# onolab-tmu/overiva

Measured on AMD Instinct MI355X. Metric: AuxIVA iterations/sec (2048 bins x 4000 frames x 8 mics), higher is better.
Workload: dtype f32

## Files before the change

include/overiva_hip.h:

```cpp
#ifndef OVERIVA_HIP_H
#define OVERIVA_HIP_H

#ifdef __cplusplus
extern "C" {
#endif

#define OIVA_OK 0
#define OIVA_ERR_ARG (-1)
#define OIVA_ERR_HIP (-2)
#define OIVA_ERR_STATE (-3)
#define OIVA_ERR_NUMERIC (-4)

#define OIVA_MODEL_LAPLACE 0
#define OIVA_MODEL_GAUSS 1

#define OIVA_MAX_CHANNELS 32

#define OIVA_PREC_FAST 0
#define OIVA_PREC_UPDATE_F64 1
#define OIVA_PREC_UPDATE_ROWS 2
#define OIVA_PREC_COV_F64 4
#define OIVA_PREC_PRECISE (OIVA_PREC_UPDATE_F64 | OIVA_PREC_COV_F64)

typedef struct oiva_plan oiva_plan;
// ... 49 lines not shown
int oiva_plan_save_w(oiva_plan *p);
int oiva_plan_restore_w(oiva_plan *p);

int oiva_plan_iterate_timed(oiva_plan *p, int n, float *total_ms, float *per_kernel_ms);
#define OIVA_N_STAGES 4

int oiva_plan_get_cov_splits(oiva_plan *p, int *nsplit);
int oiva_plan_set_cov_splits(oiva_plan *p, int nsplit);
int oiva_plan_set_cov_quad(oiva_plan *p, int enable, int *active);
int oiva_plan_set_pow_splits(oiva_plan *p, int nsplit);
int oiva_plan_set_cov_hmfma(oiva_plan *p, int enable);
int oiva_plan_set_fuse_cov_update(oiva_plan *p, int enable, int *active);
int oiva_plan_set_power_reverse(oiva_plan *p, int enable);
int oiva_plan_set_x_resident_mb(oiva_plan *p, double mb);
int oiva_plan_get_x_resident(oiva_plan *p, int *n16, int *nt, int *reason);
int oiva_plan_use_graph(oiva_plan *p, int enable);
int oiva_plan_set_precision(oiva_plan *p, int flags);

struct oiva_xchg;
#define OIVA_RESIDENT_INFO 12
#define OIVA_RESIDENT_PHASES 8
int oiva_plan_set_resident(oiva_plan *p, int enable);
int oiva_plan_resident_info(oiva_plan *p, int *info );
int oiva_plan_resident_phases(oiva_plan *p, double *phase_us , int *n_iter);
int oiva_plan_resident_debug(oiva_plan *p, int timeout_ms, int stall_block);
int oiva_plan_resident_debug_from(oiva_plan *p, int timeout_ms, int stall_block, int first_stalled_iteration);
int oiva_plan_resident_loopback(oiva_plan *p, int world);
#define OIVA_RESIDENT_STAMPS 16
int oiva_plan_resident_trace(oiva_plan *p, int enable, unsigned long long *stamps_host, int *n_wg, int *n_iter);
int oiva_plan_resident_connect(oiva_plan *p, struct oiva_xchg *x);
// ... 5 lines not shown
int oiva_test_set_rinv(oiva_plan *p, const float *rinv_host );
int oiva_test_get_rinv(oiva_plan *p, float *rinv_host , float *wscale_host );
int oiva_test_run_weighted_cov(oiva_plan *p);
int oiva_test_get_v(oiva_plan *p, void *V_host , int f64);
int oiva_test_run_update(oiva_plan *p);
int oiva_test_get_what(oiva_plan *p, void *What_host , int f64);
int oiva_test_set_what(oiva_plan *p, const void *What_host, int f64);
int oiva_test_run_power(oiva_plan *p, float *p_host );
int oiva_test_get_ppart(oiva_plan *p, float *parts_host, int *nparts);
int oiva_test_power_order(int nsplit, int tcp, int cov_splits, int cov_tc, int *order);
int oiva_test_time_stage(oiva_plan *p, int stage, int reps, float *avg_ms);
int oiva_test_live_buffers(long long *count, long long *bytes);
int oiva_test_x_policy(int T, int F, int M, int cov_tc, int pow_tcp, double budget_mb, int *out, signed char *cov_walk, signed char *pow_walk);
int oiva_test_x_choice(int T, int F, int M, int prec_flags, int cov_kind, int cov_tc, int pow_kind, int pow_tcp, double budget_mb, int from_env,
                       int *out, double *budget_used);
int oiva_test_kernel_choice(int device, int T, int F, int F_total, int M, int K, int prec_flags, int quad_on, int hmfma_on,
                            int cov_splits_req, int pow_splits_req, int *out);

#define OIVA_OGIVE_DEMIX 0
#define OIVA_OGIVE_MIX 1
#define OIVA_OGIVE_SWITCHING 2
int oiva_plan_ogive_begin(oiva_plan *p, int update_mode, int model);
int oiva_plan_ogive_iterate(oiva_plan *p, int first_epoch, int n, double step_size, double tol, int *epochs_run,
                            int *converged, double *max_delta);

typedef struct oiva_batch oiva_batch;
int oiva_batch_create(oiva_batch **out, int device, int B, int T, int F, int M, int K, int model, void *stream);
int oiva_batch_destroy(oiva_batch *b);
int oiva_batch_set_x_host(oiva_batch *b, const void *X_host, int f64);
int oiva_batch_set_x_dev(oiva_batch *b, const void *X_dev);
// ... 148 lines not shown
```

overiva_amd/_lib.py:

```python
import ctypes as C
import os

import numpy as np

_PKG = os.path.dirname(os.path.abspath(__file__))
LIB_PATH = os.environ.get("OIVA_LIB") or os.path.join(_PKG, "liboveriva_hip.so")

OK, ERR_ARG, ERR_HIP, ERR_STATE, ERR_NUMERIC = 0, -1, -2, -3, -4
MODEL_IDS = {"laplace": 0, "gauss": 1}
N_STAGES = 4
PREC_FAST, PREC_UPDATE_F64, PREC_UPDATE_ROWS, PREC_COV_F64 = 0, 1, 2, 4
PREC_PRECISE = PREC_UPDATE_F64 | PREC_COV_F64
PREC_MIXED = PREC_UPDATE_F64
PREC_BY_NAME = {"fast": PREC_FAST, "mixed": PREC_MIXED, "precise": PREC_PRECISE}
STAGE_NAMES = ("demix_power", "activation", "weighted_cov", "ip_update")


class HipLibraryMissing(ImportError):
    pass


class HipError(RuntimeError):
    """a HIP runtime call failed inside the library"""

# ... 36 lines not shown
    "oiva_xchg_destroy": [_vp],
    "oiva_plan_get_w": [_vp, _vp, _i],
    "oiva_plan_sync": [_vp],
    "oiva_plan_save_w": [_vp],
    "oiva_plan_restore_w": [_vp],
    "oiva_plan_iterate_timed": [_vp, _i, _fp, _fp],
    "oiva_plan_get_cov_splits": [_vp, C.POINTER(_i)],
    "oiva_plan_set_cov_splits": [_vp, _i],
    "oiva_plan_set_cov_quad": [_vp, _i, C.POINTER(_i)],
    "oiva_plan_set_pow_splits": [_vp, _i],
    "oiva_plan_set_cov_hmfma": [_vp, _i],
    "oiva_plan_set_fuse_cov_update": [_vp, _i, C.POINTER(_i)],
    "oiva_plan_set_power_reverse": [_vp, _i],
    "oiva_plan_set_x_resident_mb": [_vp, C.c_double],
    "oiva_plan_get_x_resident": [_vp, C.POINTER(_i), C.POINTER(_i), C.POINTER(_i)],
    "oiva_plan_use_graph": [_vp, _i],
    "oiva_plan_set_precision": [_vp, _i],
    "oiva_plan_set_resident": [_vp, _i],
    "oiva_plan_resident_info": [_vp, C.POINTER(_i)],
    "oiva_plan_resident_phases": [_vp, C.POINTER(C.c_double), C.POINTER(_i)],
    "oiva_plan_resident_debug": [_vp, _i, _i],
    "oiva_plan_resident_debug_from": [_vp, _i, _i, _i],
    "oiva_plan_resident_loopback": [_vp, _i],
    "oiva_plan_fused_connect": [_vp, _vp],
    "oiva_plan_fused_loopback": [_vp, _i],
    "oiva_plan_fused_debug": [_vp, _i, _i],
    "oiva_plan_resident_connect": [_vp, _vp],
    "oiva_plan_resident_trace": [_vp, _i, _vp, C.POINTER(_i), C.POINTER(_i)],
    "oiva_plan_set_resident_splits": [_vp, _i],
    "oiva_test_set_rinv": [_vp, _vp],
    "oiva_test_get_rinv": [_vp, _vp, _vp],
    "oiva_test_run_weighted_cov": [_vp],
    "oiva_test_get_v": [_vp, _vp, _i],
    "oiva_test_run_update": [_vp],
    "oiva_test_get_what": [_vp, _vp, _i],
    "oiva_test_set_what": [_vp, _vp, _i],
    "oiva_test_run_power": [_vp, _vp],
    "oiva_test_get_ppart": [_vp, _vp, C.POINTER(_i)],
    "oiva_test_power_order": [_i, _i, _i, _i, C.POINTER(_i)],
    "oiva_test_x_choice": [_i] * 8 + [C.c_double, _i, C.POINTER(_i), C.POINTER(C.c_double)],
    "oiva_test_x_policy": [_i, _i, _i, _i, _i, C.c_double, C.POINTER(_i), _vp, _vp],
    "oiva_test_time_stage": [_vp, _i, _i, _fp],
    "oiva_test_live_buffers": [C.POINTER(C.c_longlong), C.POINTER(C.c_longlong)],
    "oiva_test_kernel_choice": [_i] * 11 + [C.POINTER(_i)],
    "oiva_plan_ogive_begin": [_vp, _i, _i],
    "oiva_plan_ogive_iterate": [_vp, _i, _i, C.c_double, C.c_double, C.POINTER(_i), C.POINTER(_i), C.POINTER(C.c_double)],
    "oiva_batch_create": [C.POINTER(_vp), _i, _i, _i, _i, _i, _i, _i, _vp],
    "oiva_batch_destroy": [_vp],
    "oiva_batch_set_x_host": [_vp, _vp, _i],
    "oiva_batch_set_x_dev": [_vp, _vp],
    "oiva_batch_covariance": [_vp],
    "oiva_batch_set_w": [_vp, _vp, _i],
    "oiva_batch_set_w_eig": [_vp],
    "oiva_batch_iterate": [_vp, _i],
    "oiva_batch_demix": [_vp, _vp, _i, _i],
# ... 206 lines not shown
```

overiva_amd/csrc/kernel_choice.h:

```cpp
#pragma once
#include <algorithm>
#include <functional>

#include "overiva_hip.h"

namespace oiva {

inline int ceil_div(int a, int b) { return (a + b - 1) / b; }
inline int round_up(int a, int b) { return (a + b - 1) / b * b; }

constexpr int kNarrowMax = 16;
constexpr int kWideMax = OIVA_MAX_CHANNELS;

constexpr int kBinsPerWave = 16;
constexpr int kPhasesPerWave = 4;
constexpr int kBlock = 256;
constexpr int kWaves = kBlock / 64;

enum class CovKind { Lane, Pair32, Pair64, Quad, Half16, Hmfma, Half16F64, Hmfma64, Mfma, Wide };
enum class PowKind { Lane, Mfma, Lds, Wide };
constexpr int kCovKinds = 10, kPowKinds = 4;
static_assert((int)CovKind::Wide + 1 == kCovKinds && (int)PowKind::Wide + 1 == kPowKinds, "one traits row per kind");

struct CovGeom {
    int nsplit;
    int tc;
    int kc;
    int nbg;
    CovKind kind = CovKind::Lane;
    int pad = 0;
    int part32 = 0;
    int xplain = 16;
};
constexpr int kPowOrderMaxSplits = 64;
struct PowOrder {
    int cs = 0;
    int q = 0;
    int first[kPowOrderMaxSplits + 1] = {};
};
inline PowOrder make_pow_order(int n, int tcp, int cs, int ctc) {
    PowOrder o;
    if (cs < 1 || cs > kPowOrderMaxSplits || ctc < 1 || tcp < 1 || n < 1) return o;
    o.cs = cs;
    for (int s = 0; s < cs; ++s) {
        const long long c = (long long)s * ctc / tcp;
        o.first[s] = c < n ? (int)c : n;
    }
// ... 29 lines not shown
};
inline XPolicy choose_x_policy(double budget_mb, int T, int F, int M, bool cov_f64, const CovGeom& cg, const PowGeom& pg) {
    XPolicy x;
    if (!(budget_mb > 0.)) return x;
    const double frame_bytes = (double)F * M * 8., budget = budget_mb * 1e6;
    x.why = XReason::Fits, x.n16 = kXPeriod;
    if (frame_bytes * T <= budget) return x;
    x.why = XReason::Kernels, x.n16 = 0;
    if (cg.kind != CovKind::Lane || pg.kind != PowKind::Lane || cov_f64 || M != 8) return x;
    x.why = XReason::Geometry;
    if (cg.tc % kXGroup != 0 || pg.tcp % 4 != 0 || pg.tcp > cg.tc) return x;
    x.why = XReason::Share, x.nt = true;
    x.n16 = std::min(kXPeriod - 1, (int)(budget * kXPeriod / (frame_bytes * T)));
    return x;
}

enum class Partials { F64, Acc, F32IfPart32 };
struct CovTraits {
    bool (*supported)(int M, int K);
    int (*sources)(int K);
    int bins;
    int quantum;
    Partials partials;
    int launches;
    bool padded_x;
    bool quad_switch;
    bool fusable;
    bool update_arith;
    CovKind unit;
};
// ... 218 lines not shown
```

overiva_amd/csrc/kernels_cov.hip:

```cpp

#include <cstdint>
#include <cstdlib>

#include "oiva_device.h"
#include "cov_arith.h"

namespace oiva {
namespace {

constexpr int kCovUnroll = 2;
constexpr int kChunk = 16;
constexpr int kLdsStride = kBlock + 1;

template <int M, int KC, typename ACC, typename At>
__device__ __forceinline__ void reduce_and_store_at(At&& at, ACC* lds, double* __restrict__ Vpart, int F, int K, int k0) {
    constexpr int NA = M * M;
    constexpr int NACC = NA * KC;
    const int tid = threadIdx.x;
    const int bb = tid >> 4, aa = tid & 15;
    const int fo = blockIdx.x * kBinsPerWave + bb;
    double* out = Vpart + (((size_t)blockIdx.y * F + fo) * K + k0) * NA;
#pragma unroll
    for (int r0 = 0; r0 < NACC; r0 += kChunk) {
        __syncthreads();
// ... 93 lines not shown
                }
            }
#pragma unroll
            for (int c = 0; c < M; ++c) {
                ar[c] = (ACC)xr[u][c];
                ai[c] = (ACC)xi[u][c];
            }
            accumulate<M, KC, UNIT, ACC>(acc, ar, ai, w);
        }
    }

    reduce_and_store<M, KC, ACC>(acc, lds, Vpart, F, K, k0);
}

constexpr int kDmaStages = 4;

#ifdef OIVA_COVDMA_TRACE
__device__ long long g_cd_trace[8 * 2048];
#define CD_STAMP(slot)                                                                                                            \
    do {                                                                                                                          \
        if (threadIdx.x == 0 && blockIdx.z == 0) g_cd_trace[(blockIdx.y * gridDim.x + blockIdx.x) * 8 + (slot)] = wall_clock64(); \
    } while (0)
#else
#define CD_STAMP(slot) \
    do {               \
    } while (0)
#endif

template <int M, int KC>
__global__ __launch_bounds__(kBlock, 2) void cov_dma_kernel(const float2* __restrict__ X, const float* __restrict__ R,
                                                            float* __restrict__ wscale, int model, int raw,
                                                            double* __restrict__ Vpart, int T, int F, int K, int tc, int xplain) {
    constexpr int NA = M * M;
    constexpr int PIECES = M / 2;
    constexpr int STAGE = PIECES * 64;
    static_assert(M % 2 == 0 && (PIECES == 2 || PIECES == 4), "LDS-DMA path: M in {4, 8}");
    __shared__ float4 ring[kWaves * kDmaStages * STAGE];
    static_assert(sizeof(float4) * kWaves * kDmaStages * STAGE >= sizeof(float) * kChunk * kLdsStride,
                  "reduction scratch aliases the ring");

    const int tid = threadIdx.x;
    const int lane = tid & 63;
    const int wave = __builtin_amdgcn_readfirstlane(tid >> 6);
    const int b = lane & (kBinsPerWave - 1);
    const int ql = lane >> 4;
    const int q = wave * kPhasesPerWave + ql;
    const int f = blockIdx.x * kBinsPerWave + b;
    const int fc = f < F ? f : F - 1;
    const int k0 = blockIdx.z * KC;
    const int t_begin = blockIdx.y * tc;
    const int t_end = min(T, t_begin + tc);
    const int nsteps = (t_end - t_begin + 15) >> 4;

    constexpr bool kPacked = KC == 2;
    float acc[kPacked ? 1 : KC][kPacked ? 1 : NA];
    PkAcc2<M> pacc;
    if constexpr (kPacked) {
        pacc.clear();
    } else {
#pragma unroll
        for (int kk = 0; kk < KC; ++kk)
#pragma unroll
            for (int a = 0; a < NA; ++a) acc[kk][a] = 0.f;
    }

    float ginv[KC];
    float4* wring = ring + wave * kDmaStages * STAGE;
    const unsigned rd_base = (unsigned)(uintptr_t)(wring) + lane * 16;
    const size_t frame_stride = (size_t)F * M;
    const float2* pbase = X + (size_t)fc * M;
    using Rows = XRows<M>;
    const int row_off = Rows::offset(lane, blockIdx.x * kBinsPerWave, F);
    const unsigned rd_rows = (unsigned)(uintptr_t)(wring) + Rows::slot(b, ql) * 16;
    auto plain = [&](int i) { return M != 8 || x_group_plain(kXGroup * i, xplain); };

    auto issue = [&](int i, int s) {
        if (!plain(i)) {
            Rows::issue_nt(X, frame_stride, row_off, lane, t_begin + wave * kPhasesPerWave + 16 * i, i < nsteps ? t_end : 0, T, wring + s * STAGE);
            return;
        }
        const int t = t_begin + q + 16 * i;
        const int tcl = (i < nsteps && t < t_end) ? t : T - 1;
        const float2* src = pbase + (size_t)tcl * frame_stride;
#pragma unroll
        for (int j = 0; j < PIECES; ++j)
            __builtin_amdgcn_global_load_lds((gvoid_t*)(src + 2 * j), (lvoid_t*)(wring + s * STAGE + j * 64), 16, 0, 0);
    };
    const float m0 = ql == 0 ? 1.f : 0.f, m1 = ql == 1 ? 1.f : 0.f, m2 = ql == 2 ? 1.f : 0.f, m3 = ql == 3 ? 1.f : 0.f;
    auto consume = [&](int i, int s) {
        const int tw = min(t_begin + wave * kPhasesPerWave + 16 * i, T);
        const float* rp = R + (size_t)tw * K;
        float w[KC];
#pragma unroll
        for (int kk = 0; kk < KC; ++kk) {
            const int k = k0 + kk < K ? k0 + kk : K - 1;
            const float r = m0 * rp[k] + m1 * rp[K + k] + m2 * rp[2 * K + k] + m3 * rp[3 * K + k];
            const float live = (t_begin + wave * kPhasesPerWave + 16 * i + ql < t_end && k0 + kk < K) ? 1.f : 0.f;
            w[kk] = activation_weight(r, ginv[kk]) * live;
        }
        float4 v[PIECES];
        if (plain(i))
            ring_read<PIECES, (kDmaStages - 1) * PIECES>(rd_base + s * STAGE * 16, v);
        else
            ring_read_rows<PIECES, (kDmaStages - 1) * PIECES>(rd_rows + s * STAGE * 16, v);
#if defined(OIVA_COVDMA_ABLATE) && (OIVA_COVDMA_ABLATE & 1)
        if constexpr (kPacked) {
            if (v[0].x == 12345.f) pacc.add(reinterpret_cast<const v2f(&)[M]>(v), v2f{w[0], w[1]});
            return;
        }
#endif
        if constexpr (kPacked) {
            v2f x[M];
#pragma unroll
            for (int j = 0; j < PIECES; ++j) {
                x[2 * j] = v2f{v[j].x, v[j].y};
                x[2 * j + 1] = v2f{v[j].z, v[j].w};
            }
            pacc.add(x, v2f{w[0], w[1]});
        } else {
            float xr[M], xi[M];
#pragma unroll
            for (int j = 0; j < PIECES; ++j) {
                xr[2 * j] = v[j].x;
                xi[2 * j] = v[j].y;
                xr[2 * j + 1] = v[j].z;
                xi[2 * j + 1] = v[j].w;
            }
            accumulate<M, KC, false, float>(acc, xr, xi, w);
        }
    };

    CD_STAMP(0);
    issue(0, 0);
    issue(1, 1);
    issue(2, 2);
#pragma unroll
    for (int kk = 0; kk < KC; ++kk) {
        const int k = k0 + kk;
        ginv[kk] = 1.f;
        if (raw & 1) continue;
#if defined(OIVA_COVDMA_ABLATE) && (OIVA_COVDMA_ABLATE & 4)
        const float gamma = R[k < K ? k : K - 1] + 1.f;
#else
        const float gamma = (float)gamma_of(R, T, K, k < K ? k : K - 1);
#endif
        ginv[kk] = 1.f / gamma;
        if (blockIdx.x == 0 && blockIdx.y == 0 && threadIdx.x == 0 && k < K && wscale != nullptr)
            wscale[k] = model == OIVA_MODEL_LAPLACE ? gamma : sqrtf(gamma);
    }

    CD_STAMP(1);
    int i = 0;
    for (; i + 4 <= nsteps; i += 4) {
        issue(i + 3, 3); consume(i, 0);
        issue(i + 4, 0); consume(i + 1, 1);
        issue(i + 5, 1); consume(i + 2, 2);
        issue(i + 6, 2); consume(i + 3, 3);
    }
    if (i < nsteps) { issue(i + 3, 3); consume(i, 0); }
    if (i + 1 < nsteps) { issue(i + 4, 0); consume(i + 1, 1); }
    if (i + 2 < nsteps) { issue(i + 5, 1); consume(i + 2, 2); }
    CD_STAMP(2);
    asm volatile("s_waitcnt vmcnt(0)" ::: "memory");
    CD_STAMP(3);
#if defined(OIVA_COVDMA_ABLATE) && (OIVA_COVDMA_ABLATE & 2)
    if constexpr (kPacked) {
        if (pacc.at(0) == 12345.f) Vpart[0] = 1.;
        return;
    }
#endif
    if constexpr (kPacked)
        reduce_and_store_at<M, KC, float>([&](int e) { return pacc.at(e); }, reinterpret_cast<float*>(ring), Vpart, F, K, k0);
    else
        reduce_and_store<M, KC, float>(acc, reinterpret_cast<float*>(ring), Vpart, F, K, k0);
    CD_STAMP(4);
}

template <typename ACC>
using CovKernel = void (*)(const float2*, const float*, float*, int, int, double*, int, int, int, int, int);

template <int M, typename ACC, typename Fn>
hipError_t dispatch_kc(int kc, bool unit, Fn&& fn) {
    constexpr int kRegs = M * M * (int)(sizeof(ACC) / 4);
    if (unit) return kc == 1 ? fn((CovKernel<ACC>)cov_kernel<M, 1, true, ACC>, 1) : hipErrorInvalidValue;
    if constexpr ((M == 4 || M == 8) && sizeof(ACC) == 4) {
        switch (kc) {
            case 1:
                return fn((CovKernel<ACC>)cov_dma_kernel<M, 1>, 1);
            case 2:
                if constexpr (kRegs * 2 <= 144) return fn((CovKernel<ACC>)cov_dma_kernel<M, 2>, 2);
                break;
            case 4:
                if constexpr (kRegs * 4 <= 144) return fn((CovKernel<ACC>)cov_dma_kernel<M, 4>, 4);
                break;
        }
        return hipErrorInvalidValue;
    }
    switch (kc) {
// ... 4 lines not shown
            break;
        case 4:
            if constexpr (kRegs * 4 <= 144) return fn((CovKernel<ACC>)cov_kernel<M, 4, false, ACC>, 4);
            break;
        case 3:
            if constexpr (M == 7 && sizeof(ACC) == 4) return fn((CovKernel<ACC>)cov_kernel<M, 3, false, ACC>, 3);
            break;
        case 5:
            if constexpr (M == 5 && sizeof(ACC) == 4) return fn((CovKernel<ACC>)cov_kernel<M, 5, false, ACC>, 5);
            break;
    }
    return hipErrorInvalidValue;
}

template <typename ACC, typename Fn>
hipError_t dispatch_cov(int M, int kc, bool unit, Fn&& fn) {
    switch (M) {
        case 1: return dispatch_kc<1, ACC>(kc, unit, fn);
        case 2: return dispatch_kc<2, ACC>(kc, unit, fn);
        case 3: return dispatch_kc<3, ACC>(kc, unit, fn);
        case 4: return dispatch_kc<4, ACC>(kc, unit, fn);
        case 5: return dispatch_kc<5, ACC>(kc, unit, fn);
        case 6: return dispatch_kc<6, ACC>(kc, unit, fn);
        case 7: return dispatch_kc<7, ACC>(kc, unit, fn);
        case 8: return dispatch_kc<8, ACC>(kc, unit, fn);
    }
    return hipErrorInvalidValue;
}

}

__global__ __launch_bounds__(kBlock) void pad_channels_kernel(const float2* __restrict__ X, float2* __restrict__ Xpad, long long n, int M) {
    const long long e = (long long)blockIdx.x * kBlock + threadIdx.x;
    if (e >= n) return;
    const long long tf = e / (M + 1);
    const int c = (int)(e - tf * (M + 1));
    Xpad[e] = c < M ? X[tf * M + c] : make_float2(0.f, 0.f);
}

hipError_t launch_pad_channels(hipStream_t s, const float2* X, float2* Xpad, long long n_tf, int M) {
// ... 17 lines not shown
            return e != hipSuccess ? e : launch_cov_hmfma(s, Xv, Wt, V64, T, F, Mp, M, K, g);
        }
        case CovKind::Half16F64: return launch_cov_half16_f64(s, Xv, R, Wt, wscale, model, raw, V64, T, F, Mp, M, K, g);
        case CovKind::Hmfma64: {
            const hipError_t e = launch_cov_half16_weights_f64(s, R, Wt, wscale, model, raw, T, K);
            return e != hipSuccess ? e : launch_cov_hmfma64(s, Xv, reinterpret_cast<const double*>(Wt), V64, T, F, Mp, M, K, g);
        }
        case CovKind::Quad: return launch_cov_quad(s, Xv, R, Wt, wscale, model, raw, V64, T, F, Mp, M, K, g);
        case CovKind::Mfma: return launch_cov_mfma(s, X, R, Wt, wscale, model, raw, Vpart, f64, T, F, M, K, g.nsplit, g.tc);
        case CovKind::Pair32: return launch_cov_pair32(s, X, R, Wt, wscale, model, raw, V64, T, F, M, K, g);
        case CovKind::Pair64: return launch_cov_pair64(s, X, R, Wt, wscale, model, raw, V64, T, F, M, K, g);
        case CovKind::Lane: break;
    }
    const int kc = R == nullptr ? 1 : g.kc;
    if (f64)
        return dispatch_cov<double>(M, kc, R == nullptr, [&](CovKernel<double> kern, int KC) {
            kern<<<dim3(g.nbg, g.nsplit, (K + KC - 1) / KC), dim3(kBlock), 0, s>>>(X, R, wscale, model, raw,
                                                                                 static_cast<double*>(Vpart), T, F, K, g.tc, g.xplain);
            return hipGetLastError();
        });
    return dispatch_cov<float>(M, kc, R == nullptr, [&](CovKernel<float> kern, int KC) {
        return launch_dominant(kern, dim3(g.nbg, g.nsplit, (K + KC - 1) / KC), dim3(kBlock), 0, s, X, R, wscale, model, raw,
                               static_cast<double*>(Vpart), T, F, K, g.tc, g.xplain);
    });
}

hipError_t cov_blocks_per_cu(int M, int kc, bool f64, int* n) {
    if (f64)
        return dispatch_cov<double>(M, kc, false, [&](CovKernel<double> kern, int) {
            return hipOccupancyMaxActiveBlocksPerMultiprocessor(n, kern, kBlock, 0);
        });
    return dispatch_cov<float>(M, kc, false, [&](CovKernel<float> kern, int) {
        return hipOccupancyMaxActiveBlocksPerMultiprocessor(n, kern, kBlock, 0);
    });
}

#ifdef OIVA_COVDMA_TRACE
extern "C" int oiva_debug_covdma_trace(long long* out) { return (int)hipMemcpyFromSymbol(out, HIP_SYMBOL(g_cd_trace), sizeof(g_cd_trace)); }
#endif

}
```

overiva_amd/csrc/oiva_internal.h:

```cpp
#pragma once
#include <hip/hip_runtime.h>
#include <hip/hip_ext.h>

#include <string>

#include "kernel_choice.h"
#include "overiva_hip.h"

namespace oiva {

int fail_with(int code, const std::string& msg);
int xchg_peers(oiva_xchg* x, char** peers, int* rank, int* world, size_t* slot_bytes);

__host__ __device__ inline int herm_pair_index(int M, int c, int d) {
    return M + 2 * (c * M - (c * (c + 1)) / 2 + (d - c - 1));
}

__host__ __device__ inline size_t rsum_offset_floats(int T, int K) { return (((size_t)T + kPhasesPerWave) * K + 1) & ~(size_t)1; }
__host__ __device__ inline int rsum_blocks(int T) { return (T + kBlock - 1) / kBlock; }
__host__ __device__ inline size_t r_buffer_bytes(int T, int K) {
    return rsum_offset_floats(T, K) * sizeof(float) + (size_t)rsum_blocks(T) * K * sizeof(double);
}

struct KernelTimer {
// ... 33 lines not shown
hipError_t launch_cov_quad(hipStream_t s, const float2* X, const float* R, float* Wt, float* wscale, int model, int raw,
                           double* Vpart, int T, int F, int M, int Mv, int K, const CovGeom& g);
hipError_t launch_cov_weights(hipStream_t s, const float* R, float* Wt, float* wscale, int model, int raw, int T, int K, int Kp);
hipError_t launch_cov_pair64(hipStream_t s, const float2* X, const float* R, float* Wt, float* wscale, int model, int raw,
                             double* Vpart, int T, int F, int M, int K, const CovGeom& g);
hipError_t launch_cov_pair32(hipStream_t s, const float2* X, const float* R, float* Wt, float* wscale, int model, int raw,
                             double* Vpart, int T, int F, int M, int K, const CovGeom& g);
hipError_t launch_cov_half16(hipStream_t s, const float2* X, const float* R, float* Wt, float* wscale, int model, int raw,
                             double* Vpart, int T, int F, int M, int Mv, int K, const CovGeom& g);
hipError_t launch_cov_half16_weights(hipStream_t s, const float* R, float* Wt, float* wscale, int model, int raw, int T, int K);
hipError_t launch_cov_half16_weights_f64(hipStream_t s, const float* R, float* Wt, float* wscale, int model, int raw, int T, int K);
hipError_t launch_cov_hmfma(hipStream_t s, const float2* X, const float* Wt, double* Vpart, int T, int F, int M, int Mv, int K, const CovGeom& g);
hipError_t launch_cov_hmfma64(hipStream_t s, const float2* X, const double* Wt, double* Vpart, int T, int F, int M, int Mv, int K, const CovGeom& g);
hipError_t launch_cov_half16_f64(hipStream_t s, const float2* X, const float* R, float* Wt, float* wscale, int model, int raw,
                                 double* Vpart, int T, int F, int M, int Mv, int K, const CovGeom& g);
hipError_t cov_blocks_per_cu(int M, int kc, bool f64, int* n);

hipError_t launch_power(hipStream_t s, const float2* X, const float2* Xpad, const float2* What, float* Ppart, int T, int F, int M,
                        int K, const PowGeom& g);
hipError_t launch_power_mfma(hipStream_t s, const float2* X, const float2* What, float* Ppart, int T, int F, int M, int Mp, int K);
hipError_t launch_power_lds(hipStream_t s, const float2* X, const float2* What, float* Ppart, int T, int F, int M, int K);
hipError_t pow_blocks_per_cu(int M, int kp, int tcp, int* n);

constexpr int kCanonBlocks = 8;
hipError_t launch_activation_xchg(hipStream_t s, const float* parts, int nparts, char* const* gath, int rank, int world, int loopback,
                                  int nblk_own, int nblk_peer, unsigned* epochs, unsigned* ctrl, long long timeout_ticks, float* R, int T, int K,
                                  int model, int F_total);
hipError_t launch_activation(hipStream_t s, const float* parts, int nparts, float* R, int T, int K, int model,
                             int F_total);
hipError_t launch_sum_parts(hipStream_t s, const void* parts, bool f64, int nparts, double* out, long long n, double scale);

// ... 324 lines not shown
```

overiva_amd/csrc/plan.hip:

```cpp
#include <algorithm>
#include <cmath>
#include <cstdint>
#include <cstdlib>
#include <cstring>
#include <mutex>
#include <string>
#include <vector>

#include "host_io.h"
#include "host_util.h"
#include "oiva_internal.h"
#include "resident.h"

using namespace oiva;

namespace {

constexpr int kGraphBatch = 8;
constexpr int kGraphMaxIters = 32;
constexpr int kGraphCache = 6;

}

struct oiva_plan {
// ... 16 lines not shown
    void* Wwide = nullptr;
    float* R = nullptr;
    float* wscale = nullptr;
    float* Spart = nullptr;
    float2* Y = nullptr;
    double2* scratch_c = nullptr;
    double* scratch_p = nullptr;

    CovGeom cov{};
    bool cov_quad_on = true;
    bool cov_hmfma_on = true;
    bool fuse_cov_update = false;
    int power_reverse = 1;
    int pow_splits_req = 0;
    double x_resident_mb = kXResidentDefaultMB;
    CovGeom stg{};
    PowGeom pw{};
    int n_cu = 256;
    int vpart_splits_alloc = 0;

    bool have_x = false, have_cx = false, have_w = false;
    bool pad_valid = false;
    bool wscale_pending = false;
    int raw_weights = 0;
    int prec = 0;
    bool upd_f64() const { return prec & OIVA_PREC_UPDATE_F64; }
    bool cov_f64() const { return prec & OIVA_PREC_COV_F64; }
    bool vpart_f64() const { return partials_f64(cov, cov_f64()); }
    int use_graph = 0;
    OgiveState og{};
// ... 108 lines not shown

size_t vpart_floats(const oiva_plan* p, int nsplit) { return (size_t)nsplit * p->F * p->K * p->M * p->M; }

int ensure_vpart(oiva_plan* p) {
    if (p->cov.nsplit > p->vpart_splits_alloc) {
        p->mem.release(&p->Vpart);
        OIVA_TRY_HIP(p->mem.take_one(&p->Vpart, (vpart_floats(p, p->cov.nsplit) + 2) * sizeof(double)));
        p->vpart_splits_alloc = p->cov.nsplit;
    }
    return OIVA_OK;
}

XPolicy x_policy(const oiva_plan* p) { return choose_x_policy(p->x_resident_mb, p->T, p->F, p->M, p->cov_f64(), p->cov, p->pw); }
CovGeom cov_geom_now(const oiva_plan* p) {
    CovGeom g = p->cov;
    g.xplain = x_policy(p).xplain();
    return g;
}

int stage_power(oiva_plan* p) {
    PowGeom g = p->pw;
    g.xplain = x_policy(p).xplain();
    g.xctc = p->cov.tc;
    if (p->power_reverse) {
        g.rev = 1;
        if (g.rounds > 1 || p->power_reverse > 1) g.ord = make_pow_order(g.nsplit, g.tcp, p->cov.nsplit, p->cov.tc);
    }
    OIVA_TRY_HIP(launch_power(p->stream, p->X, p->X_pad && p->pad_valid ? p->X_pad : nullptr, p->What, p->Ppart, p->T, p->F, p->M, p->K, g));
    return OIVA_OK;
}
int stage_activation(oiva_plan* p, const float* parts, int nparts) {
// ... 313 lines not shown
        const hipError_t ep = p->mem.take_one(&p->X_pad, (size_t)T * F * (M + 1) * sizeof(float2));
        if (ep != hipSuccess) {
            oiva_plan_destroy(p);
            return fail_with(OIVA_ERR_HIP, std::string("allocation of the padded copy of X failed: ") + hipGetErrorString(ep));
        }
    }
    {
        const char* v = std::getenv("OIVA_COV_HMFMA");
        p->cov_hmfma_on = !(v && v[0] == '0');
        const char* u = std::getenv("OIVA_COV_UPDATE");
        p->fuse_cov_update = u && u[0] == '1';
        const char* r = std::getenv("OIVA_POWER_REVERSE");
        p->power_reverse = (r && r[0] == '0') ? 0 : (r && r[0] == '2') ? 2 : 1;
        const char* x = std::getenv("OIVA_X_RESIDENT_MB");
        if (x && x[0]) p->x_resident_mb = std::atof(x);
    }
    choose_cov_geom(p, 0);
    choose_pow_geom(p, 0);
    choose_stats_geom(p);
    p->res_ok = resident_geometry(T, F, M, K, p->n_cu, 0, &p->rg);
    const size_t nTK = (size_t)T * K;
    const size_t nFMM = (size_t)F * M * M;
    DeviceArena& mem = p->mem;
    mem.take(&p->What, nFMM * sizeof(float2));
    mem.take(&p->What64, nFMM * sizeof(double2));
    mem.take(&p->Cx, nFMM * sizeof(double));
    mem.take(&p->Ppart, (size_t)p->pw.nb * nTK * sizeof(float));
    p->ppart_alloc = p->pw.nb;
    mem.take(&p->Plocal, std::max(nTK, ((size_t)T + 1) * 32) * sizeof(float));
    if (M > kNarrowMax) mem.take(&p->Wwide, nTK * sizeof(double));
// ... 588 lines not shown
}

int oiva_plan_set_x_resident_mb(oiva_plan* p, double mb) {
    OIVA_NEED(p, OIVA_ERR_ARG, "null plan");
    OIVA_NEED(mb == mb, OIVA_ERR_ARG, "the budget is not a number");
    return change_geometry(p, [&] { p->x_resident_mb = mb; choose_pow_geom(p, p->pow_splits_req); return OIVA_OK; });
}

int oiva_plan_get_x_resident(oiva_plan* p, int* n16, int* nt, int* reason) {
    OIVA_NEED(p && n16 && nt && reason, OIVA_ERR_ARG, "null argument");
    const XPolicy x = x_policy(p);
    *n16 = x.n16, *nt = x.nt ? 1 : 0, *reason = (int)x.why;
    return OIVA_OK;
}

int oiva_plan_use_graph(oiva_plan* p, int enable) {
    OIVA_NEED(p, OIVA_ERR_ARG, "null plan");
    DeviceGuard guard(p->device);
    p->use_graph = enable ? 1 : 0;
    if (!enable) return drop_graph(p);
    if (p->have_x && p->have_cx && p->have_w && (p->F == p->F_total || p->fx_on)) return build_graphs(p);
    return OIVA_OK;
}

int oiva_plan_set_precision(oiva_plan* p, int flags) {
    OIVA_NEED(p, OIVA_ERR_ARG, "null plan");
    OIVA_NEED((flags & ~(OIVA_PREC_UPDATE_F64 | OIVA_PREC_UPDATE_ROWS | OIVA_PREC_COV_F64)) == 0, OIVA_ERR_ARG, "unknown precision flag");
    return change_geometry(p, [&] {
        if ((flags & OIVA_PREC_UPDATE_F64) && p->have_w && !p->what64_valid) {
            std::vector<double2> wh;
// ... 430 lines not shown
    OIVA_NEED(cov_kind >= 0 && cov_kind < kCovKinds && pow_kind >= 0 && pow_kind < kPowKinds, OIVA_ERR_ARG, "unknown kernel kind");
    if (from_env) {
        const char* x = std::getenv("OIVA_X_RESIDENT_MB");
        budget_mb = x && x[0] ? std::atof(x) : kXResidentDefaultMB;
    }
    CovGeom cg{};
    cg.kind = (CovKind)cov_kind, cg.tc = cov_tc, cg.nsplit = ceil_div(T, cov_tc);
    PowGeom pg{};
    pg.kind = (PowKind)pow_kind, pg.tcp = pow_tcp, pg.nsplit = ceil_div(T, pow_tcp);
    const XPolicy x = choose_x_policy(budget_mb, T, F, M, (prec_flags & OIVA_PREC_COV_F64) != 0, cg, pg);
    out[0] = x.n16, out[1] = x.nt ? 1 : 0, out[2] = (int)x.why;
    if (budget_used) *budget_used = budget_mb;
    return OIVA_OK;
}

int oiva_test_kernel_choice(int device, int T, int F, int F_total, int M, int K, int prec_flags, int quad_on, int hmfma_on,
                            int cov_splits_req, int pow_splits_req, int* out) {
    OIVA_NEED(out && T >= 1 && F >= 1 && F_total >= F && M >= 1 && M <= OIVA_MAX_CHANNELS && K >= 1 && K <= M, OIVA_ERR_ARG, "bad arguments");
    OIVA_NEED(cov_splits_req >= 0 && pow_splits_req >= 0, OIVA_ERR_ARG, "bad split count");
    DeviceGuard guard(device);
    oiva_plan p;
    p.device = device, p.T = T, p.F = F, p.F_total = F_total, p.M = M, p.K = K, p.prec = prec_flags;
    p.cov_quad_on = quad_on != 0, p.cov_hmfma_on = hmfma_on != 0;
    hipDeviceProp_t prop;
    if (hipGetDeviceProperties(&prop, device) == hipSuccess && prop.multiProcessorCount > 0) p.n_cu = prop.multiProcessorCount;
    int asked[2] = {-1, -1};
    const ChoiceIn c = choice_in(&p);
    const CovGeom g = choose_cov(c, device_occupancy(asked), cov_splits_req);
    const PowGeom w = choose_pow(c, device_occupancy(asked), pow_splits_req);
    const int o[18] = {(int)g.kind, g.nsplit, g.tc, g.kc, g.nbg, g.pad, g.part32, partials_f64(g, c.cov_f64) ? 1 : 0, (int)traits(g.kind).unit,
// ... 7 lines not shown
```

overiva_amd/plan.py:

```python
import ctypes as C

import numpy as np

from . import _lib


def _is_f64(a):
    if a.dtype == np.complex128:
        return 1
    if a.dtype == np.complex64:
        return 0
    raise TypeError(f"complex64 or complex128 expected, got {a.dtype}")


class DeviceX:

    def __init__(self, ptr, shape, owner=None, host_dtype=np.complex64):
        self.ptr = int(ptr)
        self.shape = tuple(int(v) for v in shape)
        self.owner = owner
        self.dtype = np.dtype(host_dtype)
        self.ndim = 3


# ... 163 lines not shown
        _lib.check(self.lib.oiva_plan_set_pow_splits(self.h, int(n)))

    def set_power_reverse(self, enable=True):
        _lib.check(self.lib.oiva_plan_set_power_reverse(self.h, int(enable)))

    X_RESIDENT_REASONS = ("off", "fits", "kernels", "geometry", "share")

    def set_x_resident_mb(self, mb):
        _lib.check(self.lib.oiva_plan_set_x_resident_mb(self.h, float(mb)))

    def x_resident(self):
        n16, nt, why = C.c_int(), C.c_int(), C.c_int()
        _lib.check(self.lib.oiva_plan_get_x_resident(self.h, C.byref(n16), C.byref(nt), C.byref(why)))
        return n16.value, bool(nt.value), self.X_RESIDENT_REASONS[why.value]

    def use_graph(self, enable=True):
        _lib.check(self.lib.oiva_plan_use_graph(self.h, 1 if enable else 0))

    def set_precision(self, mode="fast", row_layout=False):
        flags = _lib.PREC_BY_NAME[mode] if isinstance(mode, str) else int(mode)
        if row_layout:
            flags |= _lib.PREC_UPDATE_ROWS
        _lib.check(self.lib.oiva_plan_set_precision(self.h, flags))

    RESIDENT_INFO = ("qualifies", "enabled", "bin_groups", "frame_splits", "frames_per_split", "frames_per_lane",
                     "frames_in_registers", "lds_bytes", "last_give_up_code", "launches", "fallbacks", "x_bytes_per_cu")
    RESIDENT_PHASES = ("demix_power", "parts", "activation", "cov_accumulate", "cov_reduce", "wait_partials", "ip_update", "wait_w")

    def set_resident(self, enable=True):
        _lib.check(self.lib.oiva_plan_set_resident(self.h, 1 if enable else 0))
# ... 113 lines not shown
```

Baseline: 5670.

## Add row-form LDS-DMA covariance kernel with shallower ring for streamed X

Adds a row-layout variant of the DMA covariance kernel for M=8 that always uses the row issue/read path, with plain and nontemporal issue variants, and a configurable ring depth that defaults to 2 stages instead of 4. The variant is selected by default whenever the X-residency policy streams part of X. It removes the per-step branch between the lane and row layouts. The smaller ring cuts LDS use, which may raise occupancy, at the cost of fewer loads in flight to hide memory latency.

```diff
diff --git a/include/overiva_hip.h b/include/overiva_hip.h
--- a/include/overiva_hip.h
+++ b/include/overiva_hip.h
@@ -87,6 +87,8 @@
 int oiva_plan_set_power_reverse(oiva_plan *p, int enable);
 int oiva_plan_set_x_resident_mb(oiva_plan *p, double mb);
 int oiva_plan_get_x_resident(oiva_plan *p, int *n16, int *nt, int *reason);
+int oiva_plan_set_cov_rows(oiva_plan *p, int enable);
+int oiva_plan_get_cov_rows(oiva_plan *p, int *rows);
 int oiva_plan_use_graph(oiva_plan *p, int enable);
 int oiva_plan_set_precision(oiva_plan *p, int flags);
 
@@ -122,6 +124,9 @@
 int oiva_test_x_policy(int T, int F, int M, int cov_tc, int pow_tcp, double budget_mb, int *out, signed char *cov_walk, signed char *pow_walk);
 int oiva_test_x_choice(int T, int F, int M, int prec_flags, int cov_kind, int cov_tc, int pow_kind, int pow_tcp, double budget_mb, int from_env,
                        int *out, double *budget_used);
+int oiva_test_cov_rows(int T, int F, int M, int prec_flags, int cov_kind, int cov_tc, int pow_kind, int pow_tcp, double budget_mb, int rows_on,
+                       int *rows);
+int oiva_test_cov_blocks_per_cu(int M, int kc, int rows, int *n);
 int oiva_test_kernel_choice(int device, int T, int F, int F_total, int M, int K, int prec_flags, int quad_on, int hmfma_on,
                             int cov_splits_req, int pow_splits_req, int *out);
 
diff --git a/overiva_amd/_lib.py b/overiva_amd/_lib.py
--- a/overiva_amd/_lib.py
+++ b/overiva_amd/_lib.py
@@ -74,6 +74,8 @@
     "oiva_plan_set_power_reverse": [_vp, _i],
     "oiva_plan_set_x_resident_mb": [_vp, C.c_double],
     "oiva_plan_get_x_resident": [_vp, C.POINTER(_i), C.POINTER(_i), C.POINTER(_i)],
+    "oiva_plan_set_cov_rows": [_vp, _i],
+    "oiva_plan_get_cov_rows": [_vp, C.POINTER(_i)],
     "oiva_plan_use_graph": [_vp, _i],
     "oiva_plan_set_precision": [_vp, _i],
     "oiva_plan_set_resident": [_vp, _i],
@@ -99,6 +101,8 @@
     "oiva_test_get_ppart": [_vp, _vp, C.POINTER(_i)],
     "oiva_test_power_order": [_i, _i, _i, _i, C.POINTER(_i)],
     "oiva_test_x_choice": [_i] * 8 + [C.c_double, _i, C.POINTER(_i), C.POINTER(C.c_double)],
+    "oiva_test_cov_rows": [_i] * 8 + [C.c_double, _i, C.POINTER(_i)],
+    "oiva_test_cov_blocks_per_cu": [_i, _i, _i, C.POINTER(_i)],
     "oiva_test_x_policy": [_i, _i, _i, _i, _i, C.c_double, C.POINTER(_i), _vp, _vp],
     "oiva_test_time_stage": [_vp, _i, _i, _fp],
     "oiva_test_live_buffers": [C.POINTER(C.c_longlong), C.POINTER(C.c_longlong)],
diff --git a/overiva_amd/csrc/kernel_choice.h b/overiva_amd/csrc/kernel_choice.h
--- a/overiva_amd/csrc/kernel_choice.h
+++ b/overiva_amd/csrc/kernel_choice.h
@@ -31,6 +31,7 @@
     int pad = 0;
     int part32 = 0;
     int xplain = 16;
+    int rows = 0;
 };
 constexpr int kPowOrderMaxSplits = 64;
 struct PowOrder {
@@ -90,6 +91,8 @@
     x.n16 = std::min(kXPeriod - 1, (int)(budget * kXPeriod / (frame_bytes * T)));
     return x;
 }
+
+constexpr bool cov_rows_form(const XPolicy& x, bool rows_on) { return rows_on && x.nt; }
 
 enum class Partials { F64, Acc, F32IfPart32 };
 struct CovTraits {
diff --git a/overiva_amd/csrc/kernels_cov.hip b/overiva_amd/csrc/kernels_cov.hip
--- a/overiva_amd/csrc/kernels_cov.hip
+++ b/overiva_amd/csrc/kernels_cov.hip
@@ -131,6 +131,10 @@
 }
 
 constexpr int kDmaStages = 4;
+#ifndef OIVA_COV_ROW_STAGES
+#define OIVA_COV_ROW_STAGES 2
+#endif
+constexpr int kCovRowStages = OIVA_COV_ROW_STAGES;
 
 #ifdef OIVA_COVDMA_TRACE
 __device__ long long g_cd_trace[8 * 2048];
@@ -144,7 +148,7 @@
     } while (0)
 #endif
 
-template <int M, int KC>
+template <int M, int KC, bool ROWS = false, int S = ROWS ? kCovRowStages : kDmaStages>
 __global__ __launch_bounds__(kBlock, 2) void cov_dma_kernel(const float2* __restrict__ X, const float* __restrict__ R,
                                                             float* __restrict__ wscale, int model, int raw,
                                                             double* __restrict__ Vpart, int T, int F, int K, int tc, int xplain) {
@@ -152,8 +156,9 @@
     constexpr int PIECES = M / 2;
     constexpr int STAGE = PIECES * 64;
     static_assert(M % 2 == 0 && (PIECES == 2 || PIECES == 4), "LDS-DMA path: M in {4, 8}");
-    __shared__ float4 ring[kWaves * kDmaStages * STAGE];
-    static_assert(sizeof(float4) * kWaves * kDmaStages * STAGE >= sizeof(float) * kChunk * kLdsStride,
+    static_assert(S >= 2 && S <= 4 && (!ROWS || M == 8), "S - 1 steps in flight; the row form exists where the policy streams");
+    __shared__ float4 ring[kWaves * S * STAGE];
+    static_assert(sizeof(float4) * kWaves * S * STAGE >= sizeof(float) * kChunk * kLdsStride,
                   "reduction scratch aliases the ring");
 
     const int tid = threadIdx.x;
@@ -182,7 +187,7 @@
     }
 
     float ginv[KC];
-    float4* wring = ring + wave * kDmaStages * STAGE;
+    float4* wring = ring + wave * S * STAGE;
     const unsigned rd_base = (unsigned)(uintptr_t)(wring) + lane * 16;
     const size_t frame_stride = (size_t)F * M;
     const float2* pbase = X + (size_t)fc * M;
@@ -192,16 +197,24 @@
     auto plain = [&](int i) { return M != 8 || x_group_plain(kXGroup * i, xplain); };
 
     auto issue = [&](int i, int s) {
-        if (!plain(i)) {
-            Rows::issue_nt(X, frame_stride, row_off, lane, t_begin + wave * kPhasesPerWave + 16 * i, i < nsteps ? t_end : 0, T, wring + s * STAGE);
-            return;
-        }
-        const int t = t_begin + q + 16 * i;
-        const int tcl = (i < nsteps && t < t_end) ? t : T - 1;
-        const float2* src = pbase + (size_t)tcl * frame_stride;
-#pragma unroll
-        for (int j = 0; j < PIECES; ++j)
-            __builtin_amdgcn_global_load_lds((gvoid_t*)(src + 2 * j), (lvoid_t*)(wring + s * STAGE + j * 64), 16, 0, 0);
+        if constexpr (ROWS) {
+            const int t0 = t_begin + wave * kPhasesPerWave + 16 * i, t_lim = i < nsteps ? t_end : 0;
+            if (plain(i))
+                Rows::template issue<0>(X, frame_stride, row_off, lane, t0, t_lim, T, wring + s * STAGE);
+            else
+                Rows::template issue<2>(X, frame_stride, row_off, lane, t0, t_lim, T, wring + s * STAGE);
+        } else {
+            if (!plain(i)) {
+                Rows::issue_nt(X, frame_stride, row_off, lane, t_begin + wave * kPhasesPerWave + 16 * i, i < nsteps ? t_end : 0, T, wring + s * STAGE);
+                return;
+            }
+            const int t = t_begin + q + 16 * i;
+            const int tcl = (i < nsteps && t < t_end) ? t : T - 1;
+            const float2* src = pbase + (size_t)tcl * frame_stride;
+#pragma unroll
+            for (int j = 0; j < PIECES; ++j)
+                __builtin_amdgcn_global_load_lds((gvoid_t*)(src + 2 * j), (lvoid_t*)(wring + s * STAGE + j * 64), 16, 0, 0);
+        }
     };
     const float m0 = ql == 0 ? 1.f : 0.f, m1 = ql == 1 ? 1.f : 0.f, m2 = ql == 2 ? 1.f : 0.f, m3 = ql == 3 ? 1.f : 0.f;
     auto consume = [&](int i, int s) {
@@ -216,10 +229,14 @@
             w[kk] = activation_weight(r, ginv[kk]) * live;
         }
         float4 v[PIECES];
-        if (plain(i))
-            ring_read<PIECES, (kDmaStages - 1) * PIECES>(rd_base + s * STAGE * 16, v);
-        else
-            ring_read_rows<PIECES, (kDmaStages - 1) * PIECES>(rd_rows + s * STAGE * 16, v);
+        if constexpr (ROWS) {
+            ring_read_rows<PIECES, (S - 1) * PIECES>(rd_rows + s * STAGE * 16, v);
+        } else {
+            if (plain(i))
+                ring_read<PIECES, (S - 1) * PIECES>(rd_base + s * STAGE * 16, v);
+            else
+                ring_read_rows<PIECES, (S - 1) * PIECES>(rd_rows + s * STAGE * 16, v);
+        }
 #if defined(OIVA_COVDMA_ABLATE) && (OIVA_COVDMA_ABLATE & 1)
         if constexpr (kPacked) {
             if (v[0].x == 12345.f) pacc.add(reinterpret_cast<const v2f(&)[M]>(v), v2f{w[0], w[1]});
@@ -248,9 +265,14 @@
     };
 
     CD_STAMP(0);
-    issue(0, 0);
-    issue(1, 1);
-    issue(2, 2);
+    if constexpr (!ROWS) {
+        issue(0, 0);
+        issue(1, 1);
+        issue(2, 2);
+    } else {
+#pragma unroll
+        for (int u = 0; u < S - 1; ++u) issue(u, u);
+    }
 #pragma unroll
     for (int kk = 0; kk < KC; ++kk) {
         const int k = k0 + kk;
@@ -268,15 +290,32 @@
 
     CD_STAMP(1);
     int i = 0;
-    for (; i + 4 <= nsteps; i += 4) {
-        issue(i + 3, 3); consume(i, 0);
-        issue(i + 4, 0); consume(i + 1, 1);
-        issue(i + 5, 1); consume(i + 2, 2);
-        issue(i + 6, 2); consume(i + 3, 3);
-    }
-    if (i < nsteps) { issue(i + 3, 3); consume(i, 0); }
-    if (i + 1 < nsteps) { issue(i + 4, 0); consume(i + 1, 1); }
-    if (i + 2 < nsteps) { issue(i + 5, 1); consume(i + 2, 2); }
+    if constexpr (!ROWS) {
+        static_assert(ROWS || S == 4, "the lane form's loop is unrolled over its four stages by hand");
+        for (; i + 4 <= nsteps; i += 4) {
+            issue(i + 3, 3); consume(i, 0);
+            issue(i + 4, 0); consume(i + 1, 1);
+            issue(i + 5, 1); consume(i + 2, 2);
+            issue(i + 6, 2); consume(i + 3, 3);
+        }
+        if (i < nsteps) { issue(i + 3, 3); consume(i, 0); }
+        if (i + 1 < nsteps) { issue(i + 4, 0); consume(i + 1, 1); }
+        if (i + 2 < nsteps) { issue(i + 5, 1); consume(i + 2, 2); }
+    } else {
+        for (; i + S <= nsteps; i += S) {
+#pragma unroll
+            for (int u = 0; u < S; ++u) {
+                issue(i + u + S - 1, (u + S - 1) % S);
+                consume(i + u, u);
+            }
+        }
+#pragma unroll
+        for (int u = 0; u < S - 1; ++u)
+            if (i + u < nsteps) {
+                issue(i + u + S - 1, (u + S - 1) % S);
+                consume(i + u, u);
+            }
+    }
     CD_STAMP(2);
     asm volatile("s_waitcnt vmcnt(0)" ::: "memory");
     CD_STAMP(3);
@@ -297,8 +336,15 @@
 using CovKernel = void (*)(const float2*, const float*, float*, int, int, double*, int, int, int, int, int);
 
 template <int M, typename ACC, typename Fn>
-hipError_t dispatch_kc(int kc, bool unit, Fn&& fn) {
+hipError_t dispatch_kc(int kc, bool unit, bool rows, Fn&& fn) {
     constexpr int kRegs = M * M * (int)(sizeof(ACC) / 4);
+    if (rows) {
+        if constexpr (M == 8 && sizeof(ACC) == 4) {
+            if (!unit && kc == 1) return fn((CovKernel<ACC>)cov_dma_kernel<M, 1, true>, 1);
+            if (!unit && kc == 2) return fn((CovKernel<ACC>)cov_dma_kernel<M, 2, true>, 2);
+        }
+        return hipErrorInvalidValue;
+    }
     if (unit) return kc == 1 ? fn((CovKernel<ACC>)cov_kernel<M, 1, true, ACC>, 1) : hipErrorInvalidValue;
     if constexpr ((M == 4 || M == 8) && sizeof(ACC) == 4) {
         switch (kc) {
@@ -333,16 +379,16 @@
 }
 
 template <typename ACC, typename Fn>
-hipError_t dispatch_cov(int M, int kc, bool unit, Fn&& fn) {
+hipError_t dispatch_cov(int M, int kc, bool unit, bool rows, Fn&& fn) {
     switch (M) {
-        case 1: return dispatch_kc<1, ACC>(kc, unit, fn);
-        case 2: return dispatch_kc<2, ACC>(kc, unit, fn);
-        case 3: return dispatch_kc<3, ACC>(kc, unit, fn);
-        case 4: return dispatch_kc<4, ACC>(kc, unit, fn);
-        case 5: return dispatch_kc<5, ACC>(kc, unit, fn);
-        case 6: return dispatch_kc<6, ACC>(kc, unit, fn);
-        case 7: return dispatch_kc<7, ACC>(kc, unit, fn);
-        case 8: return dispatch_kc<8, ACC>(kc, unit, fn);
+        case 1: return dispatch_kc<1, ACC>(kc, unit, rows, fn);
+        case 2: return dispatch_kc<2, ACC>(kc, unit, rows, fn);
+        case 3: return dispatch_kc<3, ACC>(kc, unit, rows, fn);
+        case 4: return dispatch_kc<4, ACC>(kc, unit, rows, fn);
+        case 5: return dispatch_kc<5, ACC>(kc, unit, rows, fn);
+        case 6: return dispatch_kc<6, ACC>(kc, unit, rows, fn);
+        case 7: return dispatch_kc<7, ACC>(kc, unit, rows, fn);
+        case 8: return dispatch_kc<8, ACC>(kc, unit, rows, fn);
     }
     return hipErrorInvalidValue;
 }
@@ -390,23 +436,23 @@
     }
     const int kc = R == nullptr ? 1 : g.kc;
     if (f64)
-        return dispatch_cov<double>(M, kc, R == nullptr, [&](CovKernel<double> kern, int KC) {
+        return dispatch_cov<double>(M, kc, R == nullptr, g.rows != 0, [&](CovKernel<double> kern, int KC) {
             kern<<<dim3(g.nbg, g.nsplit, (K + KC - 1) / KC), dim3(kBlock), 0, s>>>(X, R, wscale, model, raw,
                                                                                  static_cast<double*>(Vpart), T, F, K, g.tc, g.xplain);
             return hipGetLastError();
         });
-    return dispatch_cov<float>(M, kc, R == nullptr, [&](CovKernel<float> kern, int KC) {
+    return dispatch_cov<float>(M, kc, R == nullptr, g.rows != 0, [&](CovKernel<float> kern, int KC) {
         return launch_dominant(kern, dim3(g.nbg, g.nsplit, (K + KC - 1) / KC), dim3(kBlock), 0, s, X, R, wscale, model, raw,
                                static_cast<double*>(Vpart), T, F, K, g.tc, g.xplain);
     });
 }
 
-hipError_t cov_blocks_per_cu(int M, int kc, bool f64, int* n) {
+hipError_t cov_blocks_per_cu(int M, int kc, bool f64, int* n, bool rows) {
     if (f64)
-        return dispatch_cov<double>(M, kc, false, [&](CovKernel<double> kern, int) {
+        return dispatch_cov<double>(M, kc, false, rows, [&](CovKernel<double> kern, int) {
             return hipOccupancyMaxActiveBlocksPerMultiprocessor(n, kern, kBlock, 0);
         });
-    return dispatch_cov<float>(M, kc, false, [&](CovKernel<float> kern, int) {
+    return dispatch_cov<float>(M, kc, false, rows, [&](CovKernel<float> kern, int) {
         return hipOccupancyMaxActiveBlocksPerMultiprocessor(n, kern, kBlock, 0);
     });
 }
diff --git a/overiva_amd/csrc/oiva_internal.h b/overiva_amd/csrc/oiva_internal.h
--- a/overiva_amd/csrc/oiva_internal.h
+++ b/overiva_amd/csrc/oiva_internal.h
@@ -71,7 +71,7 @@
 hipError_t launch_cov_hmfma64(hipStream_t s, const float2* X, const double* Wt, double* Vpart, int T, int F, int M, int Mv, int K, const CovGeom& g);
 hipError_t launch_cov_half16_f64(hipStream_t s, const float2* X, const float* R, float* Wt, float* wscale, int model, int raw,
                                  double* Vpart, int T, int F, int M, int Mv, int K, const CovGeom& g);
-hipError_t cov_blocks_per_cu(int M, int kc, bool f64, int* n);
+hipError_t cov_blocks_per_cu(int M, int kc, bool f64, int* n, bool rows = false);
 
 hipError_t launch_power(hipStream_t s, const float2* X, const float2* Xpad, const float2* What, float* Ppart, int T, int F, int M,
                         int K, const PowGeom& g);
diff --git a/overiva_amd/csrc/plan.hip b/overiva_amd/csrc/plan.hip
--- a/overiva_amd/csrc/plan.hip
+++ b/overiva_amd/csrc/plan.hip
@@ -54,6 +54,7 @@
     int power_reverse = 1;
     int pow_splits_req = 0;
     double x_resident_mb = kXResidentDefaultMB;
+    bool cov_rows_on = true;
     CovGeom stg{};
     PowGeom pw{};
     int n_cu = 256;
@@ -192,7 +193,9 @@
 XPolicy x_policy(const oiva_plan* p) { return choose_x_policy(p->x_resident_mb, p->T, p->F, p->M, p->cov_f64(), p->cov, p->pw); }
 CovGeom cov_geom_now(const oiva_plan* p) {
     CovGeom g = p->cov;
-    g.xplain = x_policy(p).xplain();
+    const XPolicy x = x_policy(p);
+    g.xplain = x.xplain();
+    g.rows = cov_rows_form(x, p->cov_rows_on) ? 1 : 0;
     return g;
 }
 
@@ -536,6 +539,8 @@
         p->power_reverse = (r && r[0] == '0') ? 0 : (r && r[0] == '2') ? 2 : 1;
         const char* x = std::getenv("OIVA_X_RESIDENT_MB");
         if (x && x[0]) p->x_resident_mb = std::atof(x);
+        const char* cr = std::getenv("OIVA_COV_ROWS");
+        p->cov_rows_on = !(cr && cr[0] == '0');
     }
     choose_cov_geom(p, 0);
     choose_pow_geom(p, 0);
@@ -1154,6 +1159,17 @@
     return OIVA_OK;
 }
 
+int oiva_plan_set_cov_rows(oiva_plan* p, int enable) {
+    OIVA_NEED(p, OIVA_ERR_ARG, "null plan");
+    return change_geometry(p, [&] { p->cov_rows_on = enable != 0; return OIVA_OK; });
+}
+
+int oiva_plan_get_cov_rows(oiva_plan* p, int* rows) {
+    OIVA_NEED(p && rows, OIVA_ERR_ARG, "null argument");
+    *rows = cov_geom_now(p).rows;
+    return OIVA_OK;
+}
+
 int oiva_plan_use_graph(oiva_plan* p, int enable) {
     OIVA_NEED(p, OIVA_ERR_ARG, "null plan");
     DeviceGuard guard(p->device);
@@ -1614,6 +1630,23 @@
     return OIVA_OK;
 }
 
+int oiva_test_cov_rows(int T, int F, int M, int prec_flags, int cov_kind, int cov_tc, int pow_kind, int pow_tcp, double budget_mb, int rows_on, int* rows) {
+    OIVA_NEED(rows && T >= 1 && F >= 1 && M >= 1 && cov_tc >= 1 && pow_tcp >= 1, OIVA_ERR_ARG, "bad arguments");
+    OIVA_NEED(cov_kind >= 0 && cov_kind < kCovKinds && pow_kind >= 0 && pow_kind < kPowKinds, OIVA_ERR_ARG, "unknown kernel kind");
+    CovGeom cg{};
+    cg.kind = (CovKind)cov_kind, cg.tc = cov_tc, cg.nsplit = ceil_div(T, cov_tc);
+    PowGeom pg{};
+    pg.kind = (PowKind)pow_kind, pg.tcp = pow_tcp, pg.nsplit = ceil_div(T, pow_tcp);
+    *rows = cov_rows_form(choose_x_policy(budget_mb, T, F, M, (prec_flags & OIVA_PREC_COV_F64) != 0, cg, pg), rows_on != 0) ? 1 : 0;
+    return OIVA_OK;
+}
+
+int oiva_test_cov_blocks_per_cu(int M, int kc, int rows, int* n) {
+    OIVA_NEED(n && M >= 1 && M <= 8 && kc >= 1, OIVA_ERR_ARG, "bad arguments");
+    OIVA_TRY_HIP(cov_blocks_per_cu(M, kc, false, n, rows != 0));
+    return OIVA_OK;
+}
+
 int oiva_test_kernel_choice(int device, int T, int F, int F_total, int M, int K, int prec_flags, int quad_on, int hmfma_on,
                             int cov_splits_req, int pow_splits_req, int* out) {
     OIVA_NEED(out && T >= 1 && F >= 1 && F_total >= F && M >= 1 && M <= OIVA_MAX_CHANNELS && K >= 1 && K <= M, OIVA_ERR_ARG, "bad arguments");
diff --git a/overiva_amd/plan.py b/overiva_amd/plan.py
--- a/overiva_amd/plan.py
+++ b/overiva_amd/plan.py
@@ -201,6 +201,14 @@
         _lib.check(self.lib.oiva_plan_get_x_resident(self.h, C.byref(n16), C.byref(nt), C.byref(why)))
         return n16.value, bool(nt.value), self.X_RESIDENT_REASONS[why.value]
 
+    def set_cov_rows(self, enable=True):
+        _lib.check(self.lib.oiva_plan_set_cov_rows(self.h, 1 if enable else 0))
+
+    def cov_rows(self):
+        rows = C.c_int()
+        _lib.check(self.lib.oiva_plan_get_cov_rows(self.h, C.byref(rows)))
+        return bool(rows.value)
+
     def use_graph(self, enable=True):
         _lib.check(self.lib.oiva_plan_use_graph(self.h, 1 if enable else 0))
 
```

New measurement: 5845, median of 6. +3.1%, better.
